# Nadeem202020/VisionTransformer-Intention-Prediction

Hardware: AMD Instinct MI355X
Metric: BEV samples/sec (fwd+bwd) IntentNetViT at 1/2/4/8 MI355X; attn MFMA util % (higher is better)
Workload: dtype bf16

## Files before the change

visiontransformer-intention-prediction_amd/csrc/patch_embed.hip:

```cpp
#include "patch_embed.h"
#include "panel_common.h"

#include <type_traits>

namespace ivit {
namespace {

constexpr int PE_MT = 144;
constexpr int PE_MB = PE_MT / 16;
constexpr int PE_STAGE = PE_MT * 8 * 32;
constexpr int PE_NS = 3;
constexpr int PE_BSTAGE = PE_MT * 8 * 16;
constexpr int PE_PIECES = PE_STAGE / 1024;

IVIT_DEV bf16x8 cvt8(const float4 a, const float4 b) {
  Pack8 p;
  p.u = f32x8_to_bf16x8(a, b);
  return p.v;
}

template <int NW>
__global__ __launch_bounds__(64 * NW, 1) void patch_fwd_kernel(const float* __restrict__ img, int C, int H, int W,
                                                           int Wp, int Np, int M, const u32x4* __restrict__ wpack,
                                                           const float* __restrict__ bias,
// ... 82 lines not shown
      const int t = f / PE_MB, mb = f % PE_MB;
      if (f + 3 < 2 * PE_MB) fr[(f + 3) % 4] = rdf(f + 3);
#pragma unroll
      for (int j = 0; j < NBW; ++j) {
        union { u32x4 u; bf16x8 v; } bw;
        bw.u = cur[t * NBW + j];
        acc[mb][j] = __builtin_amdgcn_mfma_f32_16x16x32_bf16(fr[f % 4], bw.v, acc[mb][j], 0, 0, 0);
      }
      if (f == 1 && kt + 1 < C) {
        convert(kt + 1);
        asm volatile("s_waitcnt lgkmcnt(0)" ::: "memory");
        if (kt + 4 < C) issue_a(kt + 4);
      }
      __builtin_amdgcn_sched_barrier(0);
    }
    asm volatile("s_waitcnt lgkmcnt(0)" ::: "memory");
  };

  issue_a(0);
  asm volatile("s_waitcnt vmcnt(0)" ::: "memory");
  convert(0);
  if (C > 1) issue_a(1);
  issue_b(0, breg[0]);
  if (C > 2) issue_a(2);
  if (C > 1) issue_b(1, breg[1]);
  if (C > 3) issue_a(3);
  for (int kt = 0; kt < C; kt += 3) {
    stage(kt, breg[0], breg[2]);
    if (kt + 1 < C) stage(kt + 1, breg[1], breg[0]);
    if (kt + 2 < C) stage(kt + 2, breg[2], breg[1]);
  }

  float bv[NBW];
#pragma unroll
  for (int j = 0; j < NBW; ++j) bv[j] = bias[(wv * NBW + j) * 16 + (lane & 15)];
#pragma unroll
  for (int mb = 0; mb < PE_MB; ++mb) {
    __builtin_amdgcn_sched_barrier(0);
#pragma unroll
    for (int i = 0; i < 4; ++i) {
      const int m = m0 + 16 * mb + 4 * (lane >> 4) + i;
      if (m >= M) continue;
      const int b = m / Np, p = m - b * Np;
      const float* pr = pos + (long)(1 + p) * D;
      float* orow = out + ((long)b * (Np + 1) + 1 + p) * D;
#pragma unroll
      for (int j = 0; j < NBW; ++j) {
        const int n = (wv * NBW + j) * 16 + (lane & 15);
        orow[n] = acc[mb][j][i] + bv[j] + pr[n];
      }
    }
  }
}

__global__ __launch_bounds__(256) void patch_pack_kernel(const float* __restrict__ w, long D, long K,
                                                         uint4* __restrict__ wp) {
  const long i = (long)blockIdx.x * 256 + threadIdx.x;
  const long NB16 = D / 16, total = (K / 32) * NB16 * 64;
  if (i >= total) return;
  const int lane = (int)(i & 63);
  const long snb = i >> 6, s = snb / NB16, nb = snb - s * NB16;
  const float* q = w + (nb * 16 + (lane & 15)) * K + s * 32 + 8 * (lane >> 4);
  wp[i] = f32x8_to_bf16x8(*(const float4*)q, *(const float4*)(q + 4));
}

__global__ __launch_bounds__(256) void pack_t_kernel(const float* __restrict__ w, long K, long N, uint4* __restrict__ wp) {
  const long i = (long)blockIdx.x * 256 + threadIdx.x;
  const long NB16 = N / 16, total = (K / 32) * NB16 * 64;
  if (i >= total) return;
  const int lane = (int)(i & 63);
  const long snb = i >> 6, s = snb / NB16, nb = snb - s * NB16;
  const long n = nb * 16 + (lane & 15), k0 = s * 32 + 8 * (lane >> 4);
  float v[8];
#pragma unroll
  for (int e = 0; e < 8; ++e) v[e] = w[(k0 + e) * N + n];
  wp[i] = make_uint4(pk_bf16(v[0], v[1]), pk_bf16(v[2], v[3]), pk_bf16(v[4], v[5]), pk_bf16(v[6], v[7]));
}

struct PackJob {
  const float* w;
  uint4* wp;
  long rows, cols;
  int tr;
};
__global__ __launch_bounds__(256) void multi_pack_kernel(const PackJob* __restrict__ jobs) {
  const PackJob j = jobs[blockIdx.y];
  const long total = j.rows * j.cols / 8;
  for (long i = (long)blockIdx.x * 256 + threadIdx.x; i < total; i += (long)gridDim.x * 256) {
    const int lane = (int)(i & 63);
    const long snb = i >> 6;
    if (!j.tr) {
      const long NB16 = j.rows / 16, s = snb / NB16, nb = snb - s * NB16;
      const float* q = j.w + (nb * 16 + (lane & 15)) * j.cols + s * 32 + 8 * (lane >> 4);
      j.wp[i] = f32x8_to_bf16x8(*(const float4*)q, *(const float4*)(q + 4));
    } else {
      const long NB16 = j.cols / 16, s = snb / NB16, nb = snb - s * NB16;
      const long n = nb * 16 + (lane & 15), k0 = s * 32 + 8 * (lane >> 4);
      float v[8];
#pragma unroll
      for (int e = 0; e < 8; ++e) v[e] = j.w[(k0 + e) * j.cols + n];
      j.wp[i] = make_uint4(pk_bf16(v[0], v[1]), pk_bf16(v[2], v[3]), pk_bf16(v[4], v[5]), pk_bf16(v[6], v[7]));
    }
  }
}

__global__ void patch_cls_kernel(float* out, long B, long Ntok, long D, const float* cls, const float* pos) {
  const long i = (long)blockIdx.x * blockDim.x + threadIdx.x;
  if (i >= B * D) return;
  const long b = i / D, d = i - b * D;
  out[b * Ntok * D + d] = cls[d] + pos[d];
}

}
}

using namespace ivit;

extern "C" long ivit_patch_weight_pack_bytes(long D, long C) { return D * C * 64 * 2; }

extern "C" int ivit_patch_weight_pack(const float* w, long D, long C, void* wpack, void* stream) {
  IVIT_CHECK_ARG(D > 0 && D % 16 == 0 && C > 0, "ivit_patch_weight_pack: D must be a positive multiple of 16");
  const long K = C * 64, n = (K / 32) * (D / 16) * 64;
  hipLaunchKernelGGL(patch_pack_kernel, dim3(ivit_cdiv(n, 256)), dim3(256), 0, ivit_stream(stream), w, D, K,
                     (uint4*)wpack);
  IVIT_LAUNCH_CHECK();
  return 0;
}

extern "C" int ivit_weight_pack_multi(long n, const void* jobs, long max_rows_cols, void* stream) {
  if (n <= 0) return 0;
  IVIT_CHECK_ARG(n < 65536 && jobs != nullptr, "ivit_weight_pack_multi: bad job table");
  int gx = ivit_cdiv(max_rows_cols / 8, 256);
  if (gx > 288) gx = 288;
  hipLaunchKernelGGL(multi_pack_kernel, dim3(gx, n), dim3(256), 0, ivit_stream(stream), (const PackJob*)jobs);
  IVIT_LAUNCH_CHECK();
  return 0;
}

extern "C" int ivit_weight_pack_t(const float* w, long K, long N, void* wpack, void* stream) {
  IVIT_CHECK_ARG(N > 0 && N % 16 == 0 && K > 0 && K % 32 == 0, "ivit_weight_pack_t: N % 16, K % 32 must be 0");
  const long n = (K / 32) * (N / 16) * 64;
  hipLaunchKernelGGL(pack_t_kernel, dim3(ivit_cdiv(n, 256)), dim3(256), 0, ivit_stream(stream), w, K, N, (uint4*)wpack);
  IVIT_LAUNCH_CHECK();
  return 0;
}

extern "C" int ivit_patch_embed_fwd_packed(const float* img, long B, long C, long H, long W, const void* wpack,
                                           const float* bias, const float* pos, const float* cls, long D,
                                           float* out, void* stream) {
  IVIT_CHECK_ARG(H % 8 == 0 && W % 8 == 0 && H > 0 && W > 0 && B > 0 && C > 0,
                 "ivit_patch_embed_fwd_packed: H, W must be positive multiples of the patch (8)");
  IVIT_CHECK_ARG(D == 384 || D == 192, "ivit_patch_embed_fwd_packed: D must be 384 or 192 (got %ld)", D);
  const long span = 1 + (PE_MT - 1 + (H / 8) * (W / 8) - 1) / ((H / 8) * (W / 8));
  IVIT_CHECK_ARG((H / 8) * (W / 8) * B < (1L << 31) && span * C * H * W * 4 < (1L << 32),
                 "ivit_patch_embed_fwd_packed: raster too large");
  IVIT_CHECK_ARG(((uintptr_t)img & 15) == 0 && ((uintptr_t)wpack & 15) == 0,
                 "ivit_patch_embed_fwd_packed: raster and packed weight must be 16-byte aligned");
  hipStream_t st = ivit_stream(stream);
  const int Wp = (int)(W / 8), Np = (int)((H / 8) * Wp), M = (int)(B * Np);
  const dim3 grid(ivit_cdiv(M, PE_MT));
  if (D == 384)
    hipLaunchKernelGGL(patch_fwd_kernel<8>, grid, dim3(512), 0, st, img, (int)C, (int)H, (int)W, Wp, Np, M,
                       (const u32x4*)wpack, bias, pos, (int)D, out);
  else
    hipLaunchKernelGGL(patch_fwd_kernel<4>, grid, dim3(256), 0, st, img, (int)C, (int)H, (int)W, Wp, Np, M,
                       (const u32x4*)wpack, bias, pos, (int)D, out);
  IVIT_LAUNCH_CHECK();
  const long Ntok = (long)Np + 1;
  hipLaunchKernelGGL(patch_cls_kernel, dim3(ivit_cdiv(B * D, 256)), dim3(256), 0, st, out, B, Ntok, D, cls, pos);
// ... 557 lines not shown
```

visiontransformer-intention-prediction_amd/ops.py:

```python
from __future__ import annotations

import ctypes

import torch
from torch.utils.weak import WeakIdKeyDictionary

from _lib import ACT_GELU, ACT_GELU_D, ACT_NONE, BF16, F32, KNOB_CONV_PANEL, dt, lib, ptr, stream, tdtype, workspace


def _code(dtype):
    return BF16 if dtype == torch.bfloat16 else F32


def cast(x, dtype):
    if x.dtype == dtype:
        return x
    y = torch.empty(x.shape, dtype=dtype, device=x.device)
    lib.ivit_cast(ptr(x), dt(x), ptr(y), dt(y), x.numel(), stream())
    return y


_SHADOWS = WeakIdKeyDictionary()


# ... 486 lines not shown
        raise ValueError(f"attn_rows: {what} index out of range [0, {hi}): min {int(v.min())}, max {int(v.max())}")
    return v


class RowRequests:
    __slots__ = ("B", "N", "idx")

    def __init__(self, sample, token, B, N, device):
        s, t = _request_index(sample, B, "sample"), _request_index(token, N, "token")
        if s.numel() != t.numel():
            raise ValueError(f"attn_rows: {s.numel()} samples for {t.numel()} tokens")
        self.B, self.N = int(B), int(N)
        self.idx = torch.stack([s, t]).to(torch.int32).to(device)


def attn_rows(qkv, B, N, H, cdt, sample, token=None, head_mean=False, prescaled=False):
    if dt(qkv) != cdt or not qkv.is_contiguous() or qkv.numel() != B * N * 3 * H * 64:
        raise ValueError(f"attn_rows: qkv {tuple(qkv.shape)} {qkv.dtype} is not a contiguous [B*N, 3*H*64] tensor of "
                         f"the compute dtype (B={B}, N={N}, H={H})")
    if prescaled and cdt != BF16:
        raise ValueError("attn_rows: prescaled Q exists on the bf16 path only")
    req = sample if isinstance(sample, RowRequests) else RowRequests(sample, token, B, N, qkv.device)
    if (req.B, req.N) != (B, N) or req.idx.device != qkv.device:
        raise ValueError(f"attn_rows: requests checked for B={req.B}, N={req.N} on {req.idx.device}")
    R = req.idx.shape[1]
    out = torch.empty((R, N) if head_mean else (R, H, N), dtype=torch.float32, device=qkv.device)
    if R == 0:
        return out
    lib.ivit_attn_rows(cdt, ptr(qkv), B, N, H, 64, int(bool(prescaled)), ptr(req.idx[0]), ptr(req.idx[1]), R,
                       int(bool(head_mean)), ptr(out), stream())
    return out


def add_act_grad(a, b=None, pre=None, row_scale=None, row_elems=1, out_dtype=None):
    out = torch.empty(a.shape, dtype=out_dtype or a.dtype, device=a.device)
    lib.ivit_add_act_grad(ptr(a), dt(a), ptr(b), dt(b) if b is not None else F32, ptr(pre),
                          dt(pre) if pre is not None else F32, ptr(row_scale), row_elems, ptr(out), dt(out),
                          a.numel(), stream())
    return out


def pack_conv(w, cdt, cout_pad=None):
    Cout, Cin, k, _ = w.shape
    cp = Cout if cout_pad is None else cout_pad
    out = torch.empty((cp, k, k, Cin), dtype=tdtype(cdt), device=w.device)
    lib.ivit_pack_conv_weight(cdt, ptr(w), Cout, Cin, k, cp, ptr(out), stream())
    return out


def pack_conv_pair(w0, w1, cdt, cout_pad):
    C0, Cin, k, _ = w0.shape
    C1 = w1.shape[0]
    out = torch.empty((cout_pad, k, k, Cin), dtype=tdtype(cdt), device=w0.device)
    lib.ivit_pack_conv_weight(cdt, ptr(w0), C0, Cin, k, C0, ptr(out), stream())
    lib.ivit_pack_conv_weight(cdt, ptr(w1), C1, Cin, k, cout_pad - C0, ptr(out[C0:]), stream())
    return out


def unpack_conv_grad(gp, Cout, Cin, k):
    out = torch.empty((Cout, Cin, k, k), dtype=torch.float32, device=gp.device)
    lib.ivit_unpack_conv_grad(ptr(gp), Cout, Cin, k, ptr(out), 0, stream())
    return out


def conv_fwd(x, B, H, W, wp, bias, cdt, out_dtype):
    Cout, k, _, Cin = wp.shape
    y = torch.empty((B * H * W, Cout), dtype=out_dtype, device=x.device)
    lib.ivit_conv_fwd(cdt, ptr(x), B, H, W, Cin, ptr(wp), ptr(bias), Cout, k, ptr(y), Cout, dt(y), stream())
    return y


def conv_panel_enabled():
    return lib.ivit_get_knob(KNOB_CONV_PANEL) != 0


def pack_conv_t(w, cdt, cout_pad=None):
    Cout, Cin, k, _ = w.shape
    cp = Cout if cout_pad is None else cout_pad
    out = torch.empty((Cin, k, k, cp), dtype=tdtype(cdt), device=w.device)
    lib.ivit_pack_conv_weight_t(cdt, ptr(w), Cout, Cin, k, cp, ptr(out), stream())
    return out


def conv_bn_fwd(x, B, H, W, wp, cdt, out_dtype, rmean, rvar, training, momentum=0.1, eps=1e-5, nbt=None):
    if not training:
        y = conv_fwd(x, B, H, W, wp, None, cdt, out_dtype)
        return y, bn_forward(y, None, None, rmean, rvar, False, momentum, eps)
    Cout, k, _, Cin = wp.shape
    y = torch.empty((B * H * W, Cout), dtype=out_dtype, device=x.device)
    mean = torch.empty((Cout,), dtype=torch.float32, device=x.device)
    invstd = torch.empty_like(mean)
    ws = workspace(lib.ivit_conv_bn_fwd_workspace(B, H, W, Cout), x.device)
    lib.ivit_conv_bn_fwd(cdt, ptr(x), B, H, W, Cin, ptr(wp), Cout, k, ptr(y), Cout, dt(y), ptr(mean), ptr(invstd),
                         ptr(rmean), ptr(rvar), momentum, eps, ptr(ws), ws.numel(), stream())
    if nbt is not None:
        nbt.add_(1)
    return y, _BNState(mean, invstd)


def conv_dgrad(dy, B, H, W, wp, cdt, out_dtype, w=None, dy_zero_pad=False):
    Cout, k, _, Cin = wp.shape
    dx = torch.empty((B * H * W, Cin), dtype=out_dtype, device=dy.device)
    if w is not None and cdt == BF16 and conv_panel_enabled():
        Cw = w.shape[0]
        cpad = (Cw + 63) // 64 * 64 if dy_zero_pad else Cw
        if (cpad % 64 == 0 and cpad <= dy.stride(0) and Cw <= Cout and Cin >= 128 and Cin % 8 == 0
                and B * H * W >= 288 and dy.stride(0) % 8 == 0):
            wt = pack_conv_t(w, cdt, cout_pad=cpad)
            lib.ivit_conv_dgrad_t(cdt, ptr(dy), dy.stride(0), B, H, W, cpad, ptr(wt), Cin, k, ptr(dx), dt(dx),
                                  stream())
            return dx
    lib.ivit_conv_dgrad(cdt, ptr(dy), dy.stride(0), B, H, W, Cout, ptr(wp), Cin, k, ptr(dx), dt(dx), stream())
    return dx


def conv_wgrad(dy, x, B, H, W, Cin, Cout, k, cdt, want_bias=False):
    gp = torch.empty((Cout, k, k, Cin), dtype=torch.float32, device=dy.device)
    db = torch.empty((Cout,), dtype=torch.float32, device=dy.device) if want_bias else None
    ws = workspace(lib.ivit_conv_wgrad_workspace(B, H, W, Cin, Cout, k), dy.device)
    lib.ivit_conv_wgrad(cdt, ptr(dy), dy.stride(0), ptr(x), B, H, W, Cin, Cout, k, ptr(gp), ptr(db), 0, ptr(ws),
                        ws.numel(), stream())
    return gp, db


class _BNState:

    def __init__(self, mean, invstd):
        self.mean, self.invstd = mean, invstd


def bn_forward(x, g, b, rmean, rvar, training, momentum=0.1, eps=1e-5, nbt=None):
    M, C = x.shape
    if training:
        mean = torch.empty((C,), dtype=torch.float32, device=x.device)
        invstd = torch.empty_like(mean)
        ws = workspace(lib.ivit_bn_workspace(M, C), x.device)
        lib.ivit_bn_stats(ptr(x), dt(x), M, C, ptr(mean), ptr(invstd), ptr(rmean), ptr(rvar), momentum, eps, ptr(ws),
                          ws.numel(), stream())
        if nbt is not None:
            nbt.add_(1)
    else:
        mean = torch.empty((C,), dtype=torch.float32, device=x.device)
        invstd = torch.empty_like(mean)
        lib.ivit_bn_eval_stats(ptr(rmean), ptr(rvar), C, eps, ptr(mean), ptr(invstd), stream())
    return _BNState(mean, invstd)


def bn_apply(x, st, g, b, out_dtype, resid=None, relu=False):
    M, C = x.shape
    y = torch.empty((M, C), dtype=out_dtype, device=x.device)
    if resid is not None:
        assert resid.dtype == out_dtype
    lib.ivit_bn_apply(ptr(x), dt(x), M, C, ptr(st.mean), ptr(st.invstd), ptr(g), ptr(b), ptr(resid), int(relu), ptr(y),
                      dt(y), stream())
    return y


def bn_backward(x, y, dy, st, g, relu, out_dtype, want_dr=False):
    M, C = x.shape
    dx = torch.empty((M, C), dtype=out_dtype, device=x.device)
    dr = torch.empty((M, C), dtype=out_dtype, device=x.device) if want_dr else None
    dg = torch.empty((C,), dtype=torch.float32, device=x.device)
    db = torch.empty_like(dg)
    ws = workspace(lib.ivit_bn_workspace(M, C), x.device)
    lib.ivit_bn_bwd(ptr(x), dt(x), ptr(y), dt(y), ptr(dy), dt(dy), M, C, ptr(st.mean), ptr(st.invstd), ptr(g),
                    int(relu), ptr(dx), dt(dx), ptr(dr), ptr(dg), ptr(db), 0, ptr(ws), ws.numel(), stream())
    return dx, dr, dg, db


class PatchEmbedGenericFn(torch.autograd.Function):

    @staticmethod
    def forward(ctx, img, w, b, pos, cls, cdt):
        B, C, H, W = img.shape
        D, P = w.shape[0], w.shape[-1]
        Np = (H // P) * (W // P)
        cols = torch.empty((B * Np, C * P * P), dtype=tdtype(cdt), device=img.device)
        lib.ivit_patch_im2col_p(ptr(img), B, C, H, W, P, ptr(cols), cdt, stream())
        y, _ = linear_fwd(cols, cast_weight(w, tdtype(cdt)).reshape(D, C * P * P), b, cdt, out_dtype=torch.float32)
        out = torch.empty((B * (Np + 1), D), dtype=torch.float32, device=img.device)
        lib.ivit_patch_tokens(ptr(y), B, Np, D, ptr(pos), ptr(cls), ptr(out), stream())
        ctx.save_for_backward(cols)
        ctx.meta = (B, Np, D, cdt, w.shape)
        return out

    @staticmethod
    def backward(ctx, dtok):
        (cols,) = ctx.saved_tensors
        B, Np, D, cdt, wshape = ctx.meta
        dtok = dtok.contiguous()
        dy = torch.empty((B * Np, D), dtype=tdtype(cdt), device=cols.device)
# ... 196 lines not shown
        return x2

    @staticmethod
    def backward(ctx, dx2):
        x, ln1, qkv, o, lse, x1, ln2, h, a, m1, r1, m2, r2, n1w, n2w, wq, wp, w1, w2, s1, s2 = ctx.saved_tensors
        B, N, H, cdt, _, win = block_meta(ctx.meta)
        cd = tdtype(cdt)
        dx2 = dx2.contiguous()
        dx2s = add_act_grad(dx2, row_scale=s2, row_elems=N * x.shape[1], out_dtype=cd)
        dh = linear_dgrad(dx2s, w2, cdt, cd, gelu_pre=h)
        dW2, db2 = linear_wgrad(dx2s, a, cdt)
        dln2 = linear_dgrad(dh, w1, cdt, torch.float32)
        dx1, dx1s, dg2, dbe2 = layernorm_bwd(x1, n2w, m2, r2, dln2, dres=dx2, dx=torch.empty_like(dx2), xs_dtype=cd,
                                             row_scale=s1, rps=N)
        dW1, db1 = linear_wgrad(dh, ln2, cdt)
        do = linear_dgrad(dx1s, wp, cdt, cd)
        dWp, dbp = linear_wgrad(dx1s, o, cdt)
        if win is not None:
            dqkv = (attn_win_bwd_q2(qkv, o, do, lse, B, N, H, win) if cdt == BF16
                    else attn_win_bwd(qkv, o, do, lse, B, N, H, cdt, win))
        elif cdt == BF16:
            dqkv = attn_bwd_q2(qkv, o, do, lse, B, N, H)
        else:
            dqkv = attn_bwd(qkv, o, do, lse, B, N, H, cdt)
        dln1 = linear_dgrad(dqkv, wq, cdt, torch.float32)
        dx0, _, dg1, dbe1 = layernorm_bwd(x, n1w, m1, r1, dln1, dres=dx1, dx=dx1)
        dWq, dbq = linear_wgrad(dqkv, ln1, cdt)
        return dx0, dg1, dbe1, dWq, dbq, dWp, dbp, dg2, dbe2, dW1, db1, dW2, db2, None, None, None


_UNIT_LN = {}


def _unit_ln_params(n, dev):
    key = (n, str(dev))
    if key not in _UNIT_LN:
        _UNIT_LN[key] = (torch.ones(n, device=dev), torch.zeros(n, device=dev))
    return _UNIT_LN[key]


_ZEROS = {}


def _zeros(n, dev):
    key = (n, str(dev))
    z = _ZEROS.get(key)
    if z is None:
        z = _ZEROS[key] = torch.zeros((n,), dtype=torch.float32, device=dev)
    return z


class NeckFn(torch.autograd.Function):

    @staticmethod
    def forward(ctx, tl, tm, meta, *params):
        (B, Hf, Wf, cdt, training, A, K, layers, names) = meta
        P = dict(zip(names, params))
        cd = tdtype(cdt)
        Np = Hf * Wf
        Ntok = Np + 1
        M = B * Np
        dev = tl.device
        rm = (Np, Ntok, 1)
        saved = {}
        Cl = P["adapter_lidar.1.weight"].shape[0]
        Cm = P["adapter_map.1.weight"].shape[0]
        cat = torch.empty((M, Cl + Cm), dtype=cd, device=dev)
        pre = torch.empty((M, Cl + Cm), dtype=cd, device=dev)
        for s, t, c0, C in (("lidar", tl, 0, Cl), ("map", tm, Cl, Cm)):
            y, mf, rf = layernorm_fwd(t, P[f"vit_{s}.norm.weight"], P[f"vit_{s}.norm.bias"], 1e-6, torch.float32,
                                      rowmap=rm, M=M)
            z, ma, ra = layernorm_fwd(y, P[f"adapter_{s}.0.weight"], P[f"adapter_{s}.0.bias"], 1e-5, cd)
            wa = cast_weight(P[f"adapter_{s}.1.weight"], cd)
            linear_fwd(z, wa, P[f"adapter_{s}.1.bias"], cdt, act=ACT_GELU, out=cat[:, c0:c0 + C],
                       pre=pre[:, c0:c0 + C])
            saved[s] = (t, y, mf, rf, z, ma, ra, wa)
        x = cat
        bns = {}
        packs = {}
        acts = []
        nbts = []
        for li in range(layers):
            p = f"fusion_block.{li}."
            w1 = pack_conv(P[p + "conv1.weight"], cdt)
            w2 = pack_conv(P[p + "conv2.weight"], cdt)
            c1, s1 = conv_bn_fwd(x, B, Hf, Wf, w1, cdt, torch.float32, P[p + "bn1.running_mean"],
                                 P[p + "bn1.running_var"], training)
            r1 = bn_apply(c1, s1, P[p + "bn1.weight"], P[p + "bn1.bias"], cd, relu=True)
            c2, s2 = conv_bn_fwd(r1, B, Hf, Wf, w2, cdt, torch.float32, P[p + "bn2.running_mean"],
                                 P[p + "bn2.running_var"], training)
            nbts += [P.get(p + "bn1.num_batches_tracked"), P.get(p + "bn2.num_batches_tracked")]
            if (p + "downsample.0.weight") in P:
                wd = pack_conv(P[p + "downsample.0.weight"], cdt)
                dd, sd = conv_bn_fwd(x, B, Hf, Wf, wd, cdt, torch.float32, P[p + "downsample.1.running_mean"],
                                     P[p + "downsample.1.running_var"], training)
                nbts.append(P.get(p + "downsample.1.num_batches_tracked"))
                idn = bn_apply(dd, sd, P[p + "downsample.1.weight"], P[p + "downsample.1.bias"], cd)
                bns[p + "ds"] = (dd, sd, idn)
                packs[p + "ds"] = wd
            else:
                idn = x
            out = bn_apply(c2, s2, P[p + "bn2.weight"], P[p + "bn2.bias"], cd, resid=idn, relu=True)
            acts.append((x, c1, s1, r1, c2, s2, out))
            packs[p + "1"], packs[p + "2"] = w1, w2
            x = out
        nbts = [t for t in nbts if t is not None]
        if training and nbts:
            torch._foreach_add_(nbts, 1)
        if A == 0:
            ctx.st = (saved, cat, pre, acts, bns, packs, None, x, 0)
            ctx.meta, ctx.P = meta, P
            return (cast(x, torch.float32) if x.dtype != torch.float32 else x.clone(),)
        Cd, Ci = A * 7, A * K
        Cp = (Cd + Ci + 7) // 8 * 8
        wd_, wi_ = P["det_head.conv.weight"], P["intention_head.conv.weight"]
        wh = (wd_, wi_)
        whp = pack_conv_pair(wd_, wi_, cdt, Cp)
        bh = torch.empty((Cp,), dtype=torch.float32, device=dev)
        bh[:Cd].copy_(P["det_head.conv.bias"])
        bh[Cd:Cd + Ci].copy_(P["intention_head.conv.bias"])
        bh[Cd + Ci:].copy_(_zeros(Cp - Cd - Ci, dev))
        hout = conv_fwd(x, B, Hf, Wf, whp, bh, cdt, torch.float32)
        cls = torch.empty((B, M // B * A, 1), dtype=torch.float32, device=dev)
        box = torch.empty((B, M // B * A, 6), dtype=torch.float32, device=dev)
        intent = torch.empty((B, M // B * A, K), dtype=torch.float32, device=dev)
        lib.ivit_split_heads(ptr(hout), Cp, M, A, K, ptr(cls), ptr(box), ptr(intent), stream())
        ctx.st = (saved, cat, pre, acts, bns, packs, (whp, wh), x, Cp)
        ctx.meta = meta
        ctx.P = P
        return cls, box, intent

    @staticmethod
    def backward(ctx, *gouts):
        (B, Hf, Wf, cdt, training, A, K, layers, names) = ctx.meta
        saved, cat, pre, acts, bns, packs, (whp, wh), x_last, Cp = ctx.st
        P = ctx.P
        cd = tdtype(cdt)
        Np = Hf * Wf
        M = B * Np
        dev = cat.device
        G = {}

        def cw(n_, dy_, x_, Cin_, Cout_, k_):
            gp_, _ = conv_wgrad(dy_, x_, B, Hf, Wf, Cin_, Cout_, k_, cdt)
            G[n_] = unpack_conv_grad(gp_, Cout_, Cin_, k_)

        if A == 0:
            dx = gouts[0].contiguous().float()
        else:
            dcls, dbox, dint = gouts
            Cq = (Cp + 63) // 64 * 64
            dh = torch.empty((M, Cq), dtype=cd, device=dev)
            lib.ivit_merge_heads_grad(ptr(dcls.contiguous()), ptr(dbox.contiguous()), ptr(dint.contiguous()), M, A,
                                      K, ptr(dh), Cq, dt(dh), stream())
            Cin = x_last.shape[1]
            Cd, Ci = A * 7, A * K

            def head_wgrad(dh, x_last):
                gp, dbh = conv_wgrad(dh, x_last, B, Hf, Wf, Cin, Cp, 3, cdt, want_bias=True)
                gw = unpack_conv_grad(gp, Cd + Ci, Cin, 3)
                return gw[:Cd], gw[Cd:], dbh[:Cd], dbh[Cd:Cd + Ci]

            for n_, g_ in zip(("det_head.conv.weight", "intention_head.conv.weight", "det_head.conv.bias",
                               "intention_head.conv.bias"), head_wgrad(dh, x_last)):
                G[n_] = g_
            dx = conv_dgrad(dh, B, Hf, Wf, whp, cdt, torch.float32, w=torch.cat(wh, 0), dy_zero_pad=True)
        for li in reversed(range(layers)):
            p = f"fusion_block.{li}."
            x, c1, s1, r1, c2, s2, out = acts[li]
            has_ds = (p + "ds") in bns
            dc2, dres, G[p + "bn2.weight"], G[p + "bn2.bias"] = bn_backward(c2, out, dx, s2, P[p + "bn2.weight"], True,
                                                                            cd, want_dr=True)
            Cm_ = c2.shape[1]
            cw(p + "conv2.weight", dc2, r1, r1.shape[1], Cm_, 3)
            dr1 = conv_dgrad(dc2, B, Hf, Wf, packs[p + "2"], cdt, torch.float32, w=P[p + "conv2.weight"])
            dc1, _, G[p + "bn1.weight"], G[p + "bn1.bias"] = bn_backward(c1, r1, dr1, s1, P[p + "bn1.weight"], True, cd)
            cw(p + "conv1.weight", dc1, x, x.shape[1], Cm_, 3)
            dxa = conv_dgrad(dc1, B, Hf, Wf, packs[p + "1"], cdt, torch.float32, w=P[p + "conv1.weight"])
            if has_ds:
                dd, sd, idn = bns[p + "ds"]
                ddd, _, G[p + "downsample.1.weight"], G[p + "downsample.1.bias"] = bn_backward(
                    dd, idn, dres, sd, P[p + "downsample.1.weight"], False, cd)
                cw(p + "downsample.0.weight", ddd, x, x.shape[1], Cm_, 1)
                dxb = conv_dgrad(ddd, B, Hf, Wf, packs[p + "ds"], cdt, torch.float32,
                                 w=P[p + "downsample.0.weight"])
            else:
                dxb = dres
            if li == 0:
                dx = add_act_grad(dxa, dxb, pre=pre, out_dtype=cd)
            else:
                dx = add_act_grad(dxa, dxb, out_dtype=torch.float32)
        dpre = dx
        Cl = P["adapter_lidar.1.weight"].shape[0]
        outs = {}
        for s, c0 in (("lidar", 0), ("map", Cl)):
            t, y, mf, rf, z, ma, ra, wa = saved[s]
            C = wa.shape[0]
            dp = dpre[:, c0:c0 + C]
            dz = linear_dgrad(dp, wa, cdt, torch.float32)
            G[f"adapter_{s}.1.weight"], G[f"adapter_{s}.1.bias"] = linear_wgrad(dp, z, cdt)
            dy, _, G[f"adapter_{s}.0.weight"], G[f"adapter_{s}.0.bias"] = layernorm_bwd(
                y, P[f"adapter_{s}.0.weight"], ma, ra, dz)
            dt_ = torch.empty_like(t)
            dt_.view(B, Np + 1, -1)[:, 0].zero_()
            _, _, G[f"vit_{s}.norm.weight"], G[f"vit_{s}.norm.bias"] = layernorm_bwd(
                t, P[f"vit_{s}.norm.weight"], mf, rf, dy, dx=dt_, rowmap=(Np, Np + 1, 1))
            outs[s] = dt_
        grads = [G.get(n) for n in names]
        del ctx.st, ctx.P
        return (outs["lidar"], outs["map"], None) + tuple(grads)


class DetLossFn(torch.autograd.Function):

    @staticmethod
    def forward(ctx, cls, box, intent, anchors, gt, ngt, gint, keep, cfg):
        B, NA = cls.shape[0], cls.shape[1]
        K = intent.shape[-1]
        G = gt.shape[1]
        dev = cls.device
        stats = torch.zeros((16,), dtype=torch.float32, device=dev)
        ws = workspace(lib.ivit_det_loss_workspace(B, NA, G), dev)
        cls, box, intent = cls.contiguous(), box.contiguous(), intent.contiguous()
        lib.ivit_det_loss_fwd(ptr(cls), ptr(box), ptr(intent), ptr(anchors), B, NA, K, ptr(gt), ptr(ngt), ptr(gint), G,
                              ptr(keep), cfg["dominant_mask"], int(cfg["downsampling"]), ptr(cfg.get("class_w")),
                              cfg["pos_thr"], cfg["neg_thr"], cfg["alpha"], cfg["gamma"], cfg["beta"], cfg["w_cls"],
                              cfg["w_box"], cfg["w_int"], int(cfg["rotated"]), ptr(stats), ptr(ws), ws.numel(),
                              stream())
        ctx.save_for_backward(cls, box, intent, keep, stats, ws)
        ctx.cfg = cfg
        ctx.shape = (B, NA, K)
        ctx.mark_non_differentiable(stats)
        ctx.set_materialize_grads(False)
        loss = stats[5:6].clone().reshape(())
        return loss, stats

    @staticmethod
    def backward(ctx, gloss, _gstats):
        cls, box, intent, keep, stats, ws = ctx.saved_tensors
        B, NA, K = ctx.shape
        cfg = ctx.cfg
        if gloss is None:
            return None, None, None, None, None, None, None, None, None
        g = gloss.reshape(1).float().contiguous()
        dcls, dbox, dint = torch.empty_like(cls), torch.empty_like(box), torch.empty_like(intent)
        lib.ivit_det_loss_bwd(ptr(cls), ptr(box), ptr(intent), B, NA, K, ptr(keep), cfg["dominant_mask"],
                              int(cfg["downsampling"]), ptr(cfg.get("class_w")), cfg["alpha"], cfg["gamma"],
                              cfg["beta"], cfg["w_cls"], cfg["w_box"], cfg["w_int"], ptr(stats), ptr(g), ptr(dcls),
                              ptr(dbox), ptr(dint), ptr(ws), ws.numel(), stream())
        return dcls, dbox, dint, None, None, None, None, None, None


class DetIouLossFn(torch.autograd.Function):

    @staticmethod
    def forward(ctx, cls, box, intent, anchors, gt, ngt, gint, keep, cfg):
        B, NA = cls.shape[0], cls.shape[1]
        K = intent.shape[-1]
        G = gt.shape[1]
        dev = cls.device
        stats = torch.zeros((16,), dtype=torch.float32, device=dev)
        ws = workspace(lib.ivit_det_loss_workspace(B, NA, G), dev)
        iws = workspace(lib.ivit_det_iou_loss_workspace(B, NA), dev)
        cls, box, intent = cls.contiguous(), box.contiguous(), intent.contiguous()
        lib.ivit_det_loss_fwd(ptr(cls), ptr(box), ptr(intent), ptr(anchors), B, NA, K, ptr(gt), ptr(ngt), ptr(gint), G,
                              ptr(keep), cfg["dominant_mask"], int(cfg["downsampling"]), ptr(cfg.get("class_w")),
                              cfg["pos_thr"], cfg["neg_thr"], cfg["alpha"], cfg["gamma"], cfg["beta"], cfg["w_cls"],
                              cfg["w_box"], cfg["w_int"], int(cfg["rotated"]), ptr(stats), ptr(ws), ws.numel(),
# ... 180 lines not shown
```

visiontransformer-intention-prediction_amd/optim.py:

```python
from __future__ import annotations

import contextlib
import ctypes
import math

import torch

import ops
from _lib import lib, ptr, stream, workspace


class _Tables:

    def __init__(self):
        self._tables = {}

    def _table(self, tensors, device):
        key = tuple(t.data_ptr() for t in tensors)
        tab = self._tables.get(key)
        if tab is None:
            tab = torch.tensor(key, dtype=torch.int64).pin_memory().to(device, non_blocking=True)
            if len(self._tables) > 64:
                self._tables.clear()
            self._tables[key] = tab
        return tab

    def _table_chunks(self, ps, device):
        key = ("chunks",) + tuple(p.numel() for p in ps)
        tab = self._tables.get(key)
        if tab is None:
            ce = lib.ivit_adamw_chunk_elems()
            rec = [(t, c) for t, p in enumerate(ps) for c in range(-(-p.numel() // ce))]
            tab = (torch.tensor(rec, dtype=torch.int32).reshape(len(rec), 2).pin_memory().to(device, non_blocking=True),
                   len(rec))
            if len(self._tables) > 64:
                self._tables.clear()
            self._tables[key] = tab
        return tab

    def _table_sizes(self, ps, device):
        key = ("sizes",) + tuple(p.numel() for p in ps)
        tab = self._tables.get(key)
        if tab is None:
            tab = torch.tensor([p.numel() for p in ps], dtype=torch.int64).pin_memory().to(device, non_blocking=True)
            self._tables[key] = tab
        return tab

    def _norm_launch(self, grads, max_norm, finite, stats):
        max_norm = float(max_norm)
        if not max_norm > 0.0:
            raise ValueError(f"max_norm must be > 0 (got {max_norm})")
        for g in grads:
            if not g.is_cuda:
                raise RuntimeError("ivit ops take device tensors (no CPU fallback)")
            if g.dtype != torch.float32 or not g.is_contiguous():
                raise TypeError("grad norm: contiguous f32 gradients required")
        if stats is not None and (stats.dtype != torch.float64 or stats.numel() < 5):
            raise TypeError("grad norm: stats is a device f64 tensor of 5 elements")
        dev = grads[0].device if grads else (finite.device if finite is not None else torch.device("cuda"))
        chunks, nch = self._table_chunks(grads, dev)
        key = ("normws", nch, str(dev))
        ws = self._tables.get(key)
        if ws is None:
            ws = self._tables[key] = workspace(lib.ivit_grad_norm_workspace(nch), dev)
        rec = torch.empty(4, dtype=torch.float32, device=dev)
        tg, sizes = (self._table(grads, dev), self._table_sizes(grads, dev)) if grads else (None, None)
        lib.ivit_grad_norm(len(grads), ptr(tg), ptr(sizes), ptr(chunks) if nch else None, nch, max_norm, ptr(finite),
                           ptr(ws), ws.numel(), ptr(rec), ptr(stats), stream())
        return GradNorm(rec)

    def _scale_launch(self, grads, coef):
        if not grads:
            return
        dev = grads[0].device
        chunks, nch = self._table_chunks(grads, dev)
        lib.ivit_grad_scale(len(grads), ptr(self._table(grads, dev)), ptr(self._table_sizes(grads, dev)),
                            ptr(chunks) if nch else None, nch, ptr(coef), stream())

    def _followers(self, ps):
        shadows, jobs, big = [], [], 0
        for p in ps:
            sh = ops.shadow_of(p)
            shadows.append(sh.data_ptr() if sh is not None else 0)
            pk, pkt = ops.packs_of(p)
            rows, cols = p.shape[0], p.numel() // p.shape[0]
            for pack, tr in ((pk, 0), (pkt, 1)):
                if pack is not None:
                    jobs.append((p.data_ptr(), pack.data_ptr(), rows, cols, tr))
                    big = max(big, rows * cols)
        return shadows, jobs, big

    def _table_ptrs(self, ptrs, device):
        key = ("ptrs",) + tuple(ptrs)
        tab = self._tables.get(key)
        if tab is None:
            tab = torch.tensor(ptrs, dtype=torch.int64).pin_memory().to(device, non_blocking=True)
            if len(self._tables) > 64:
                self._tables.clear()
            self._tables[key] = tab
        return tab

    def _table_hyper(self, runs, device):
        key = ("hyper",) + tuple(runs)
        tab = self._tables.get(key)
        if tab is None:
            rows = [(s, w) for s, w, n in runs for _ in range(n)]
            tab = torch.tensor(rows, dtype=torch.float32).reshape(len(rows), 2).pin_memory().to(device, non_blocking=True)
            if len(self._tables) > 64:
                self._tables.clear()
            self._tables[key] = tab
        return tab

    def _pack_jobs(self, jobs, device):
        key = ("packs",) + tuple(jobs)
        tab = self._tables.get(key)
        if tab is None:
            rec = []
            for w, wp, rows, cols, tr in jobs:
                rec += [w, wp, rows, cols, tr]
            tab = torch.tensor(rec, dtype=torch.int64).pin_memory().to(device, non_blocking=True)
            if len(self._tables) > 64:
                self._tables.clear()
            self._tables[key] = tab
        return tab


class GradNorm:
    __slots__ = ("record", "norm", "coef", "finite")

    def __init__(self, record):
        self.record = record
        self.norm, self.coef, self.finite = record[0], record[1], record[2]


STATS_FIELDS = ("steps", "clipped", "nonfinite", "norm_sum", "norm_max")


def _f32(x):
    return ctypes.c_float(x).value


def effective_lr(lr, lr_scale):
    return _f32(_f32(lr) * _f32(lr_scale))


class FusedAdamW(torch.optim.Optimizer, _Tables):

    def __init__(self, params, lr=1e-3, betas=(0.9, 0.999), eps=1e-8, weight_decay=1e-2, fuse_groups=False):
        super().__init__(params, dict(lr=lr, betas=betas, eps=eps, weight_decay=weight_decay))
        self.fuse_groups = bool(fuse_groups)
        self._tables = {}

    @torch.no_grad()
    def step(self, closure=None, finite=None, grad_scale=None):
        return self._step(closure, finite, grad_scale, None)

    @torch.no_grad()
    def step_ema(self, ema, closure=None, finite=None, grad_scale=None):
        return self._step(closure, finite, grad_scale, ema)

    def _step(self, closure, finite, grad_scale, ema):
        if ema is not None and ema._swapped:
            raise RuntimeError("FusedAdamW: the ModelEMA is swapped into the model (leave swapped() first)")
        loss = None
        if closure is not None:
            with torch.enable_grad():
                loss = closure()
        merged = {}
        for group in self.param_groups:
            live = [p for p in group["params"] if p.grad is not None]
            for p in live:
                if p.dtype != torch.float32 or p.grad.dtype != torch.float32 or not p.is_contiguous() \
# ... 305 lines not shown
```

Measured before the change: 193.8.

## Cache packed conv weights and refresh them inside the optimizer pack kernel

Conv weight packs (forward and transposed dgrad layouts) are now cached per parameter, keyed on tensor version and pointer, so each step no longer repacks them on the fly. The optimizer's multi-pack kernel gains conv-pack job types that rewrite the cached images right after the weight update, keeping them in sync. The cost is extra state and bookkeeping for cache invalidation, and a risk of stale packs if a weight changes outside the optimizer without a version bump.

```diff
diff --git a/visiontransformer-intention-prediction_amd/csrc/patch_embed.hip b/visiontransformer-intention-prediction_amd/csrc/patch_embed.hip
--- a/visiontransformer-intention-prediction_amd/csrc/patch_embed.hip
+++ b/visiontransformer-intention-prediction_amd/csrc/patch_embed.hip
@@ -188,9 +188,31 @@
   uint4* wp;
   long rows, cols;
   int tr;
+  int aux;
 };
+static_assert(sizeof(PackJob) == 40, "the job table is five 8-byte words per record");
+
+__device__ __forceinline__ void multi_pack_conv(const PackJob& j) {
+  const unsigned Cout = (unsigned)j.rows, Cin = (unsigned)j.cols, ks = j.aux & 255, Cpad = (unsigned)j.aux >> 8;
+  const unsigned kk = ks * ks, total = Cout * Cin * kk;
+  bf16* out = (bf16*)j.wp;
+  for (unsigned i = blockIdx.x * 256 + threadIdx.x; i < total; i += gridDim.x * 256) {
+    if (j.tr == 2) {
+      const unsigned ci = i % Cin, t = i / Cin, tap = t % kk, co = t / kk;
+      out[i] = from_f32<bf16>(j.w[(co * Cin + ci) * kk + tap]);
+    } else {
+      const unsigned co = i % Cout, t = i / Cout, tap = t % kk, ci = t / kk;
+      out[t * Cpad + co] = from_f32<bf16>(j.w[(co * Cin + ci) * kk + (kk - 1 - tap)]);
+    }
+  }
+}
+
 __global__ __launch_bounds__(256) void multi_pack_kernel(const PackJob* __restrict__ jobs) {
   const PackJob j = jobs[blockIdx.y];
+  if (j.tr >= 2) {
+    multi_pack_conv(j);
+    return;
+  }
   const long total = j.rows * j.cols / 8;
   for (long i = (long)blockIdx.x * 256 + threadIdx.x; i < total; i += (long)gridDim.x * 256) {
     const int lane = (int)(i & 63);
diff --git a/visiontransformer-intention-prediction_amd/ops.py b/visiontransformer-intention-prediction_amd/ops.py
--- a/visiontransformer-intention-prediction_amd/ops.py
+++ b/visiontransformer-intention-prediction_amd/ops.py
@@ -592,6 +592,78 @@
     return out
 
 
+_CONV_PACKS = WeakIdKeyDictionary()
+
+
+class ConvImage:
+    __slots__ = ("image", "tr", "dest", "cpad", "off")
+
+    def __init__(self, image, tr, off, cpad):
+        self.image, self.tr, self.off, self.cpad = image, tr, off, cpad
+        self.dest = image[off:] if tr == 2 else image.view(-1)[off:]
+
+
+def _conv_cacheable(w, cdt, cpad):
+    return (cdt == BF16 and w.is_cuda and w.dtype == torch.float32 and w.is_contiguous() and w.dim() == 4
+            and w.shape[2] == w.shape[3] and w.shape[2] <= 255 and w.shape[0] <= cpad
+            and cpad * w[0].numel() < 2 ** 31)
+
+
+def _conv_entry(w):
+    e, stamp = _CONV_PACKS.get(w), (w._version, w.data_ptr())
+    if e is None or e[0] != stamp:
+        e = (stamp, {})
+        _CONV_PACKS[w] = e
+    return e[1]
+
+
+def _conv_cached(ws, key, tr, cpad, build):
+    ents = [_conv_entry(t) for t in ws]
+    recs = [d.get(key) for d in ents]
+    if all(r is not None for r in recs) and all(r.image is recs[0].image for r in recs):
+        return recs[0].image
+    image = build()
+    off = 0
+    for t, d in zip(ws, ents):
+        d[key] = ConvImage(image, tr, off, cpad)
+        off += t.shape[0]
+    return image
+
+
+def conv_pack(w, cdt, cout_pad=None):
+    ws = w if isinstance(w, tuple) else (w,)
+    cp = sum(t.shape[0] for t in ws) if cout_pad is None else cout_pad
+
+    if len(ws) > 2:
+        raise ValueError("conv_pack: one weight or a pair")
+
+    def build():
+        return pack_conv(ws[0], cdt, cp) if len(ws) == 1 else pack_conv_pair(ws[0], ws[1], cdt, cp)
+
+    if not all(_conv_cacheable(t, cdt, cp) for t in ws):
+        return build()
+    return _conv_cached(ws, ("f", cp) + tuple(id(t) for t in ws), 2, cp, build)
+
+
+def conv_pack_t(w, cdt, cout_pad=None):
+    ws = w if isinstance(w, tuple) else (w,)
+    cp = sum(t.shape[0] for t in ws) if cout_pad is None else cout_pad
+
+    def build():
+        return pack_conv_t(torch.cat(ws, 0) if len(ws) > 1 else ws[0], cdt, cp)
+
+    if not all(_conv_cacheable(t, cdt, cp) for t in ws):
+        return build()
+    return _conv_cached(ws, ("t", cp) + tuple(id(t) for t in ws), 3, cp, build)
+
+
+def conv_packs_of(p):
+    e = _CONV_PACKS.get(p)
+    if e is None or e[0] != (p._version, p.data_ptr()):
+        return []
+    return list(e[1].values())
+
+
 def conv_bn_fwd(x, B, H, W, wp, cdt, out_dtype, rmean, rvar, training, momentum=0.1, eps=1e-5, nbt=None):
     if not training:
         y = conv_fwd(x, B, H, W, wp, None, cdt, out_dtype)
@@ -608,15 +680,19 @@
     return y, _BNState(mean, invstd)
 
 
-def conv_dgrad(dy, B, H, W, wp, cdt, out_dtype, w=None, dy_zero_pad=False):
+def conv_dgrad(dy, B, H, W, wp, cdt, out_dtype, w=None, dy_zero_pad=False, cached=False):
     Cout, k, _, Cin = wp.shape
     dx = torch.empty((B * H * W, Cin), dtype=out_dtype, device=dy.device)
     if w is not None and cdt == BF16 and conv_panel_enabled():
-        Cw = w.shape[0]
+        ws = w if isinstance(w, tuple) else (w,)
+        Cw = sum(t.shape[0] for t in ws)
         cpad = (Cw + 63) // 64 * 64 if dy_zero_pad else Cw
         if (cpad % 64 == 0 and cpad <= dy.stride(0) and Cw <= Cout and Cin >= 128 and Cin % 8 == 0
                 and B * H * W >= 288 and dy.stride(0) % 8 == 0):
-            wt = pack_conv_t(w, cdt, cout_pad=cpad)
+            if cached:
+                wt = conv_pack_t(w, cdt, cpad)
+            else:
+                wt = pack_conv_t(torch.cat(ws, 0) if len(ws) > 1 else ws[0], cdt, cout_pad=cpad)
             lib.ivit_conv_dgrad_t(cdt, ptr(dy), dy.stride(0), B, H, W, cpad, ptr(wt), Cin, k, ptr(dx), dt(dx),
                                   stream())
             return dx
@@ -979,8 +1055,8 @@
         nbts = []
         for li in range(layers):
             p = f"fusion_block.{li}."
-            w1 = pack_conv(P[p + "conv1.weight"], cdt)
-            w2 = pack_conv(P[p + "conv2.weight"], cdt)
+            w1 = conv_pack(P[p + "conv1.weight"], cdt)
+            w2 = conv_pack(P[p + "conv2.weight"], cdt)
             c1, s1 = conv_bn_fwd(x, B, Hf, Wf, w1, cdt, torch.float32, P[p + "bn1.running_mean"],
                                  P[p + "bn1.running_var"], training)
             r1 = bn_apply(c1, s1, P[p + "bn1.weight"], P[p + "bn1.bias"], cd, relu=True)
@@ -988,7 +1064,7 @@
                                  P[p + "bn2.running_var"], training)
             nbts += [P.get(p + "bn1.num_batches_tracked"), P.get(p + "bn2.num_batches_tracked")]
             if (p + "downsample.0.weight") in P:
-                wd = pack_conv(P[p + "downsample.0.weight"], cdt)
+                wd = conv_pack(P[p + "downsample.0.weight"], cdt)
                 dd, sd = conv_bn_fwd(x, B, Hf, Wf, wd, cdt, torch.float32, P[p + "downsample.1.running_mean"],
                                      P[p + "downsample.1.running_var"], training)
                 nbts.append(P.get(p + "downsample.1.num_batches_tracked"))
@@ -1012,7 +1088,7 @@
         Cp = (Cd + Ci + 7) // 8 * 8
         wd_, wi_ = P["det_head.conv.weight"], P["intention_head.conv.weight"]
         wh = (wd_, wi_)
-        whp = pack_conv_pair(wd_, wi_, cdt, Cp)
+        whp = conv_pack(wh, cdt, Cp)
         bh = torch.empty((Cp,), dtype=torch.float32, device=dev)
         bh[:Cd].copy_(P["det_head.conv.bias"])
         bh[Cd:Cd + Ci].copy_(P["intention_head.conv.bias"])
@@ -1061,7 +1137,7 @@
             for n_, g_ in zip(("det_head.conv.weight", "intention_head.conv.weight", "det_head.conv.bias",
                                "intention_head.conv.bias"), head_wgrad(dh, x_last)):
                 G[n_] = g_
-            dx = conv_dgrad(dh, B, Hf, Wf, whp, cdt, torch.float32, w=torch.cat(wh, 0), dy_zero_pad=True)
+            dx = conv_dgrad(dh, B, Hf, Wf, whp, cdt, torch.float32, w=wh, dy_zero_pad=True, cached=True)
         for li in reversed(range(layers)):
             p = f"fusion_block.{li}."
             x, c1, s1, r1, c2, s2, out = acts[li]
@@ -1070,17 +1146,19 @@
                                                                             cd, want_dr=True)
             Cm_ = c2.shape[1]
             cw(p + "conv2.weight", dc2, r1, r1.shape[1], Cm_, 3)
-            dr1 = conv_dgrad(dc2, B, Hf, Wf, packs[p + "2"], cdt, torch.float32, w=P[p + "conv2.weight"])
+            dr1 = conv_dgrad(dc2, B, Hf, Wf, packs[p + "2"], cdt, torch.float32, w=P[p + "conv2.weight"],
+                             cached=True)
             dc1, _, G[p + "bn1.weight"], G[p + "bn1.bias"] = bn_backward(c1, r1, dr1, s1, P[p + "bn1.weight"], True, cd)
             cw(p + "conv1.weight", dc1, x, x.shape[1], Cm_, 3)
-            dxa = conv_dgrad(dc1, B, Hf, Wf, packs[p + "1"], cdt, torch.float32, w=P[p + "conv1.weight"])
+            dxa = conv_dgrad(dc1, B, Hf, Wf, packs[p + "1"], cdt, torch.float32, w=P[p + "conv1.weight"],
+                             cached=True)
             if has_ds:
                 dd, sd, idn = bns[p + "ds"]
                 ddd, _, G[p + "downsample.1.weight"], G[p + "downsample.1.bias"] = bn_backward(
                     dd, idn, dres, sd, P[p + "downsample.1.weight"], False, cd)
                 cw(p + "downsample.0.weight", ddd, x, x.shape[1], Cm_, 1)
                 dxb = conv_dgrad(ddd, B, Hf, Wf, packs[p + "ds"], cdt, torch.float32,
-                                 w=P[p + "downsample.0.weight"])
+                                 w=P[p + "downsample.0.weight"], cached=True)
             else:
                 dxb = dres
             if li == 0:
diff --git a/visiontransformer-intention-prediction_amd/optim.py b/visiontransformer-intention-prediction_amd/optim.py
--- a/visiontransformer-intention-prediction_amd/optim.py
+++ b/visiontransformer-intention-prediction_amd/optim.py
@@ -88,6 +88,10 @@
                 if pack is not None:
                     jobs.append((p.data_ptr(), pack.data_ptr(), rows, cols, tr))
                     big = max(big, rows * cols)
+            for im in ops.conv_packs_of(p):
+                aux = p.shape[2] | im.cpad << 8
+                jobs.append((p.data_ptr(), im.dest.data_ptr(), p.shape[0], p.shape[1], im.tr | aux << 32))
+                big = max(big, 8 * p.numel())
         return shadows, jobs, big
 
     def _table_ptrs(self, ptrs, device):
```

After: 193.2. No clear change (-0.4%).
